# JunkyByte/easy_ViTPose

Measured on AMD Instinct MI355X. Metric: persons_per_sec, higher is better.
Workload: dtype fp16; 1 GPU; ViTPose-B coco K=17, batch 256 x 256x192 crops per GPU (f32 input resident in HBM) -> (y,x,conf) keypoints in HBM; global_batch=256, weights=seeded random init (no checkpoint offline)

## Files before the change

### easy_vitpose_amd/csrc/debug_taps.hip

```cpp
#include "api_internal.h"

using namespace vpi;

namespace {
vp_ctx* dbg_ctx(int device, int dtype) {
    int ndev = 0;
    if (hipGetDeviceCount(&ndev) != hipSuccess || device < 0 || device >= ndev) {
        g_create_error = "no HIP device available (no CPU fallback)";
        return nullptr;
    }
    if (hipSetDevice(device) != hipSuccess) return nullptr;
    vp_ctx* c = new vp_ctx();
    c->cfg.device_id = device;
    c->dtype = dtype == VP_DTYPE_F16 ? vp::DT_F16 : vp::DT_BF16;
    apply_gemm_tuning(c->sw);
    return c;
}
int dbg_finish(vp_ctx* c, int rc) {
    if (rc) g_create_error = c->err;
    vp_destroy(c);
    return rc;
}
int download16(vp_ctx* c, const uint16_t* d, float* out, size_t n) {
    std::vector<uint16_t> t(n);
// ... 274 lines not shown
    if ((r = dalloc(c, &dA, (size_t)M * K)) || (r = dalloc(c, &dW, wrows * K)) || (r = dalloc(c, &c->zero, (size_t)256))) return r;
    vp::fill_random16(c->dtype, dA, (size_t)M * K, 1u, nullptr);
    vp::fill_random16(c->dtype, dW, wrows * K, 2u, nullptr);
    if (flags & 64) { HIPCHK(c, hipMemset(dA, 0, (size_t)M * K * 2)); HIPCHK(c, hipMemset(dW, 0, wrows * K * 2)); }
    if (flags & 128) { HIPCHK(c, hipMemsetD16(dA, 0x3c00, (size_t)M * K)); HIPCHK(c, hipMemsetD16(dW, 0x3c00, wrows * K)); }
    std::vector<float> hb(wrows), hs(wrows), hr((size_t)M * 2);
    uint32_t lcg = 12345u;
    auto rnd = [&]() { lcg = lcg * 1664525u + 1013904223u; return (float)((lcg >> 8) & 0xffff) / 65536.f - 0.5f; };
    for (auto& v : hb) v = rnd();
    for (auto& v : hs) v = 4.f * rnd();
    for (size_t i = 0; i < (size_t)M; ++i) { hr[2 * i] = 0.2f * rnd(); hr[2 * i + 1] = 1.f + 0.4f * rnd(); }
    if ((r = upload_f32(c, &dB, hb.data(), wrows))) return r;
    vp::GemmArgs& g = rc.g;
    g.A = dA; g.W = dW; g.bias = dB; g.M = M; g.N = N; g.K = K; g.ldo = N; g.zero = c->zero; g.Kp = c->Kp;
    g.w_rows = (int)wrows;
    g.persist = (flags & 1) != 0; g.out_blocked = (flags & 2) != 0; g.a_blocked = (flags & 4) != 0; g.reverse = (flags & 8) != 0;
    if (flags & 16) {
        if ((r = upload_f32(c, &dRow, hr.data(), (size_t)M * 2)) || (r = upload_f32(c, &dS, hs.data(), wrows))) return r;
        g.rowstat = dRow; g.ln_s = dS;
    }
    if (epi == vp::EPI_BIAS || epi == vp::EPI_BIAS_GELU) {
        rc.out_bytes = MN * 2;
    } else if (epi == vp::EPI_BIAS_RESID || epi == vp::EPI_POS) {
        rc.out_bytes = MN * 4;
        const size_t na = epi == vp::EPI_BIAS_RESID ? MN : (size_t)192 * N;
        if ((r = dalloc(c, &dAux32, na))) return r;
        std::vector<float> ha(na);
        for (auto& v : ha) v = 2.f * rnd();
        HIPCHK(c, hipMemcpy(dAux32, ha.data(), na * 4, hipMemcpyHostToDevice));
        g.aux = dAux32;
    } else if (epi == vp::EPI_BIAS_RESID_LN) {
// ... 42 lines not shown
        for (size_t m = 0; m < (size_t)M; ++m)
            for (size_t k = 0; k < (size_t)K; ++k) {
                const size_t dst = ablk ? ((((m >> 6) * (K >> 6) + (k >> 6)) << 12) + ((m & 63) << 6) + (k & 63)) : m * K + k;
                ha[dst] = host_to_bits(A[m * K + k], c->dtype);
            }
        if ((r = dalloc(c, &dA, (size_t)M * K))) return dbg_finish(c, r);
        if (hipMemcpy(dA, ha.data(), ha.size() * 2, hipMemcpyHostToDevice) != hipSuccess) return dbg_finish(c, fail(c, VP_ERR_HIP, "H2D"));
    }
    size_t fin_rows = 0;
    if (epi == vp::EPI_HEATMAP) { if ((r = upload_final(c, &dW, W, N, K, &fin_rows))) return dbg_finish(c, r); }
    else if ((r = upload_mat(c, &dW, W, N, K, wrows))) return dbg_finish(c, r);
    if ((r = upload_f32(c, &dB, bias, N, wrows)) || (r = dalloc(c, &c->zero, (size_t)256))) return dbg_finish(c, r);
    vp::GemmArgs g{};
    g.A = dA; g.W = dW; g.bias = dB; g.M = M; g.N = N; g.K = K; g.ldo = N; g.zero = c->zero; g.Kp = N;
    g.w_rows = (int)wrows; g.variant = variant; g.group_m = group_m;
    g.persist = (flags & 1) != 0; g.out_blocked = oblk; g.a_blocked = ablk; g.reverse = (flags & 8) != 0;
    if (rowstat && ln_s) {
        if ((r = upload_f32(c, &dRow, rowstat, (size_t)M * 2)) || (r = upload_f32(c, &dS, ln_s, N, wrows))) return dbg_finish(c, r);
        g.rowstat = dRow; g.ln_s = dS;
    }
    size_t out_bytes = 0;
    const bool prod = epi == vp::EPI_BIAS_RESID_LN || epi == vp::EPI_POS_LN;
    if (epi == vp::EPI_BIAS || epi == vp::EPI_BIAS_GELU) out_bytes = MN * 2;
    else if (epi == vp::EPI_BIAS_RESID || epi == vp::EPI_POS || prod) out_bytes = MN * 4;
    else if (epi == vp::EPI_HEATMAP) { out_bytes = MN * 4; g.N = (int)fin_rows; g.ldo = 0; g.w_rows = (int)pad128(fin_rows); }
    else return dbg_finish(c, fail(c, VP_ERR_INVALID, "unsupported epilogue"));
    if (epi == vp::EPI_BIAS_RESID || epi == vp::EPI_POS || epi == vp::EPI_POS_LN) {
        if (!aux) return dbg_finish(c, fail(c, VP_ERR_INVALID, "aux required"));
        if ((r = upload_f32(c, &dAux32, aux, epi == vp::EPI_BIAS_RESID ? MN : (size_t)192 * N))) return dbg_finish(c, r);
        g.aux = dAux32;
    }
// ... 342 lines not shown
```

### easy_vitpose_amd/csrc/gemm.hip

```cpp
#include <cstdio>
#include <cstdlib>
#include <type_traits>
#include <utility>

#include "common.h"
#include "kernels.h"

namespace vp {

template <int BM_, int BN_, int BK_, int WM_, int WN_, int STAGES_, int PIPE_ = 0, int DIRECT_ = 0>
struct TileCfg {
    static constexpr int DIRECT = DIRECT_;
    static constexpr int BM = BM_, BN = BN_, BK = BK_, WM = WM_, WN = WN_, STAGES = STAGES_;
    static constexpr int PIPE = PIPE_;
    static constexpr int NWM = BM / WM, NWN = BN / WN, NWAVES = NWM * NWN, NT = NWAVES * 64;
    static constexpr int ROWB = BK * 2;
    static constexpr int SLOTS = ROWB / 16;
    static constexpr int RPG = 1024 / ROWB;
    static constexpr int W_BYTES = BN * ROWB, A_BYTES = BM * ROWB, STAGE_BYTES = W_BYTES + A_BYTES;
    static constexpr int LDS = STAGES * STAGE_BYTES;
    static constexpr int WP = BN / RPG / NWAVES, AP = BM / RPG / NWAVES;
    static constexpr int G = WP + AP;
    static constexpr int KK = BK / 32, TI = WN / 16, TJ = WM / 16;
    static_assert(BK == 64 || BK == 32, "BK");
// ... 21 lines not shown
}

__device__ __forceinline__ float row8_sum(float x) {
    x += __builtin_bit_cast(float, __builtin_amdgcn_update_dpp(0, __builtin_bit_cast(int, x), 0xB1, 0xF, 0xF, true));
    x += __builtin_bit_cast(float, __builtin_amdgcn_update_dpp(0, __builtin_bit_cast(int, x), 0x4E, 0xF, 0xF, true));
    x += __builtin_bit_cast(float, __builtin_amdgcn_update_dpp(0, __builtin_bit_cast(int, x), 0x141, 0xF, 0xF, true));
    return x;
}

template <class C> constexpr int epi_rows_per_pass_ln() {
    int jp = C::TJ;
    while (jp > 1 && C::NWM * jp * 16 * (C::BN * 4 + 16) + C::BM * (C::BN / 64) * 8 > C::LDS) jp /= 2;
    return jp;
}

template <int OFF> __device__ __forceinline__ void lds_read_b128(u32x4& d, uint32_t addr) {
    asm volatile("ds_read_b128 %0, %1 offset:%2" : "=v"(d) : "v"(addr), "n"(OFF));
}
template <int N> __device__ __forceinline__ void wait_lgkm() {
    asm volatile("s_waitcnt lgkmcnt(%0)" ::"n"(N));
    __builtin_amdgcn_sched_barrier(0);
}
template <int ROWB, int... Is>
__device__ __forceinline__ void lds_read_frags(u32x4* d, uint32_t addr, std::integer_sequence<int, Is...>) {
    (lds_read_b128<Is * 16 * ROWB>(d[Is], addr), ...);
}

template <int N> __device__ __forceinline__ void wait_vmcnt() {
    asm volatile("s_waitcnt vmcnt(%0)" ::"n"(N) : "memory");
}
// ... 20 lines not shown
    }
}

template <class T, class C, int J>
__device__ __forceinline__ void pipe5_half1(f32x4 (&acc)[C::TI][C::TJ], u32x4* f1) {
    if constexpr (J < C::TJ) {
        wait_lgkm<C::TJ - J - 1>();
#pragma unroll
        for (int i = 0; i < C::TI; ++i) acc[i][J] = mfma16<T>(f1[i], f1[C::TI + J], acc[i][J]);
        __builtin_amdgcn_sched_barrier(0);
        pipe5_half1<T, C, J + 1>(acc, f1);
    }
}

template <class T, int EPI_, int AMODE, class C, bool EXPERT = false>
__global__ __launch_bounds__(C::NT, 2) void gemm_kernel(GemmArgs g) {
    constexpr bool LN_PROD = (EPI_ == EPI_BIAS_RESID_LN || EPI_ == EPI_POS_LN);
    constexpr int EPI = LN_PROD ? EPI_ - 4 : EPI_;
    extern __shared__ __attribute__((aligned(16))) char smem[];
    const int tid = threadIdx.x, lane = tid & 63, wave = tid >> 6;
    const int tiles_n = (g.N + C::BN - 1) / C::BN;
    const int tiles_m = (g.M + C::BM - 1) / C::BM;
    int bid, parity = 0, split = 0;
    if (AMODE == A_DECONV && g.parity_fast) {
        const int lb = xcd_remap(blockIdx.x, tiles_m * tiles_n * 4);
        parity = lb & 3;
        bid = lb >> 2;
    } else if (EPI_ == EPI_PARTIAL) {
        const int lb = xcd_remap(blockIdx.x, tiles_m * tiles_n * g.splitk);
        split = lb / (tiles_m * tiles_n);
        bid = lb - split * (tiles_m * tiles_n);
    } else {
        bid = xcd_remap(blockIdx.x, tiles_m * tiles_n);
        if (AMODE == A_DECONV) parity = blockIdx.y;
    }
    if (g.reverse) bid = tiles_m * tiles_n - 1 - bid;
    int tm, tn;
    if (g.group_m > 1) {
        const int per_group = g.group_m * tiles_n;
        const int grp = bid / per_group, first_m = grp * g.group_m;
        const int gsz = min(tiles_m - first_m, g.group_m);
        const int r = bid - grp * per_group;
        tm = first_m + r % gsz;
        tn = r / gsz;
    } else {
        tm = bid / tiles_n;
        tn = bid - tm * tiles_n;
    }
    const int n0 = tn * C::BN, m0 = tm * C::BM;
    if constexpr (EXPERT) {
        const int e = g.expert[m0 / 192];
        g.W += (size_t)e * g.w_rows * g.K;
        g.bias += (size_t)e * g.w_rows;
    }
    const int K = g.K;
    const int klen = (EPI_ == EPI_PARTIAL) ? K / g.splitk : K;
    const int kbase = (EPI_ == EPI_PARTIAL) ? split * klen : 0;
    if constexpr (LN_PROD) {
        if (VP_STAGGER(g) > 0 && blockIdx.x < 512) {
            const int mode = VP_STAGGER(g) / 1000, n = VP_STAGGER(g) % 1000;
            const uint32_t hw = __builtin_amdgcn_s_getreg((31 << 11) | (0 << 6) | 4);
            bool late;
            if (mode == 0) late = (hw >> 1) & 1;
            else if (mode == 1) late = blockIdx.x >= 256;
            else if (mode == 3) late = (hw >> 8) & 1;
            else if (mode == 4) late = blockIdx.x & 1;
            else if (mode == 5) late = (hw >> 13) & 1;
            else late = (blockIdx.x >> 3) & 1;
            if (late) for (int i = 0; i < n; ++i) __builtin_amdgcn_s_sleep(16);
        }
    }

    const int rip = lane / C::SLOTS, pslot = lane % C::SLOTS;
    const uint16_t* wsrc[C::WP];
    const uint16_t* asrc[C::AP];
    int ai[C::AP], aj[C::AP];
    const uint16_t* W = g.W + (AMODE == A_DECONV ? (size_t)parity * g.w_parity_stride : 0);
#pragma unroll
    for (int p = 0; p < C::WP; ++p) {
        const int r = (p * C::NWAVES + wave) * C::RPG + rip;
        wsrc[p] = W + (size_t)(n0 + r) * K + swz<C::BK>(r, pslot) * 8;
    }
#pragma unroll
    for (int p = 0; p < C::AP; ++p) {
        const int r = (p * C::NWAVES + wave) * C::RPG + rip;
        int m = ((VP_ABLATE(g) & 2) ? 0 : m0) + r;
        if (m > g.M - 1) m = g.M - 1;
        const int sl = swz<C::BK>(r, pslot) * 8;
        if (AMODE == A_DENSE) {
            asrc[p] = g.a_blocked ? g.A + ((size_t)(m >> 6) * (K >> 6) << 12) + ((m & 63) << 6) + sl : g.A + (size_t)m * K + sl;
        } else {
            const int t = m / g.Win;
            ai[p] = t % g.Hin;
            aj[p] = m - t * g.Win;
            asrc[p] = g.A + (size_t)m * g.Cin + sl;
        }
    }
    auto stage = [&](int kt, int buf) {
        char* base = smem + buf * C::STAGE_BYTES + wave * 1024;
        const int k0 = kbase + kt * C::BK;
#pragma unroll
        for (int p = 0; p < C::WP; ++p) glds16(wsrc[p] + k0, base + p * (C::NWAVES * 1024));
        if (AMODE == A_DENSE) {
            const int ka = g.a_blocked ? ((k0 >> 6) << 12) + (k0 & 63) : k0;
#pragma unroll
            for (int p = 0; p < C::AP; ++p) glds16(asrc[p] + ka, base + C::W_BYTES + p * (C::NWAVES * 1024));
        } else {
            const int tap = k0 / g.Cin, c0 = k0 - tap * g.Cin;
            const int ti = tap >> 1, tj = tap & 1;
            const int pa = parity >> 1, pb = parity & 1;
            const int di = pa ? (ti ? 0 : 1) : (ti ? -1 : 0);
            const int dj = pb ? (tj ? 0 : 1) : (tj ? -1 : 0);
#pragma unroll
            for (int p = 0; p < C::AP; ++p) {
                const bool ok = (unsigned)(ai[p] + di) < (unsigned)g.Hin && (unsigned)(aj[p] + dj) < (unsigned)g.Win;
                const uint16_t* src = ok ? asrc[p] + (ptrdiff_t)(di * g.Win + dj) * g.Cin + c0 : g.zero + pslot * 8;
                glds16(src, base + C::W_BYTES + p * (C::NWAVES * 1024));
            }
        }
    };

    const int wn = wave / C::NWM, wm = wave % C::NWM;
    const int frow = lane & 15, fg = lane >> 4;
    const int foff = frow * C::ROWB + (swz<C::BK>(frow, fg) << 4);
    const int woff = wn * C::WN * C::ROWB + foff;
    const int aoff = C::W_BYTES + wm * C::WM * C::ROWB + foff;

    f32x4 acc[C::TI][C::TJ];
#pragma unroll
    for (int i = 0; i < C::TI; ++i)
#pragma unroll
        for (int j = 0; j < C::TJ; ++j) acc[i][j] = f32x4{0.f, 0.f, 0.f, 0.f};

    const int nk = klen / C::BK;
    if constexpr (C::PIPE == 2) {
        static_assert(C::KK == 1 && C::STAGES >= 3, "PIPE 2 needs BK = 32 and >= 3 stages");
        u32x4 wfA[C::TI], afA[C::TJ], wfB[C::TI], afB[C::TJ];
        auto ldfrag = [&](u32x4(&wf)[C::TI], u32x4(&af)[C::TJ], int b) {
            const char* sb = smem + b * C::STAGE_BYTES;
#pragma unroll
            for (int i = 0; i < C::TI; ++i) wf[i] = *(const u32x4*)(sb + (woff + i * 16 * C::ROWB));
#pragma unroll
            for (int j = 0; j < C::TJ; ++j) af[j] = *(const u32x4*)(sb + (aoff + j * 16 * C::ROWB));
        };
        auto settle = [&](u32x4(&wf)[C::TI], u32x4(&af)[C::TJ]) {
#pragma unroll
            for (int i = 0; i < C::TI; ++i) asm volatile("" ::"v"(wf[i]));
#pragma unroll
            for (int j = 0; j < C::TJ; ++j) asm volatile("" ::"v"(af[j]));
// ... 75 lines not shown
                for (int j = 0; j < C::TJ; ++j) acc[i][j] = mfma16<T>(wf[i], af[j], acc[i][j]);
            __builtin_amdgcn_s_setprio(0);
            asm volatile("" ::: "memory");
            __builtin_amdgcn_s_barrier();
            asm volatile("" ::: "memory");
            rbuf = (rbuf + 1) & 3;
            pbuf = (pbuf + 1) & 3;
        }
        if (!grp_b) {
            __builtin_amdgcn_s_barrier();
            asm volatile("" ::: "memory");
        }
    } else {
    constexpr int KS = (C::PIPE == 6) ? 2 : 1;
    static_assert(C::PIPE != 6 || (C::STAGES >= 4 && C::KK == 2), "PIPE 6: >= 4 stages, BK = 64");
#pragma unroll
    for (int s = 0; s < C::STAGES - KS; ++s)
        if (s < nk) stage(s, s);
    if constexpr (EPI == EPI_BIAS || EPI == EPI_BIAS_GELU) {
        if (g.ln_part) {
            float2* st = (float2*)(smem + C::LDS);
            for (int r = tid; r < C::BM; r += C::NT) {
                int m = m0 + r;
                if (m > g.M - 1) m = g.M - 1;
                const float* src = g.ln_part + (size_t)m * g.ln_tiles * 2;
                float mean = 0.f, rstd = 1.f;
                switch (g.ln_tiles) {
                    case 6: ln_merge_row<6>(src, g.ln_inv_d, mean, rstd); break;
                    case 12: ln_merge_row<12>(src, g.ln_inv_d, mean, rstd); break;
                    case 16: ln_merge_row<16>(src, g.ln_inv_d, mean, rstd); break;
                    case 20: ln_merge_row<20>(src, g.ln_inv_d, mean, rstd); break;
                    default: ln_merge(src, g.ln_tiles, g.ln_inv_d, mean, rstd);
                }
                st[r] = float2{mean, rstd};
            }
        }
    }
    int buf = 0, pbuf = C::STAGES - KS;
    for (int kt = 0; kt < nk; kt += KS) {
        if (C::STAGES > 2 * KS && kt + C::STAGES - KS <= nk) wait_vmcnt<C::G * (C::STAGES - 2 * KS)>();
        else wait_vmcnt<0>();
        __builtin_amdgcn_s_barrier();
        asm volatile("" ::: "memory");
#pragma unroll
        for (int ks = 0; ks < KS; ++ks) {
            const int pb = pbuf + ks >= C::STAGES ? pbuf + ks - C::STAGES : pbuf + ks;
            if (kt + C::STAGES - KS + ks < nk && !(VP_ABLATE(g) & 1)) stage(kt + C::STAGES - KS + ks, pb);
        }
#pragma unroll
        for (int ks = 0; ks < KS; ++ks) {
        const int cbuf = buf + ks >= C::STAGES ? buf + ks - C::STAGES : buf + ks;
        const char* sb = smem + cbuf * C::STAGE_BYTES;
        if constexpr (C::PIPE == 5) {
            static_assert(C::KK == 2 && C::TI + C::TJ <= 12 && 2 * C::TJ >= C::TI + C::TJ, "PIPE 5 schedule");
            constexpr int R = C::TI + C::TJ;
            u32x4 f0[R], f1[R];
            const uint32_t lb = (uint32_t)(size_t)(lds_ptr_t)(smem) + cbuf * C::STAGE_BYTES;
            const uint32_t wa0 = lb + woff, wa1 = lb + (woff ^ 64), aa0 = lb + aoff, aa1 = lb + (aoff ^ 64);
            lds_read_frags<C::ROWB>(f0, wa0, std::make_integer_sequence<int, C::TI>{});
            lds_read_frags<C::ROWB>(f0 + C::TI, aa0, std::make_integer_sequence<int, C::TJ>{});
            __builtin_amdgcn_s_setprio(1);
            __builtin_amdgcn_sched_barrier(0);
// ... 123 lines not shown
                float* orow = g.out2 + ((size_t)im * g.Kp + nb) * opix + px;
#pragma unroll
                for (int r = 0; r < 4; ++r)
                    if (im >= 0 && nb + r < g.Kp) orow[(size_t)r * opix] = v[r] + b2[r];
            }
        };
        for (int u = 0; u < groups; u += 2) {
            if (u + 1 < groups) ldw(wB, u + 1);
            group(wA, u);
            if (u + 1 < groups) {
                if (u + 2 < groups) ldw(wA, u + 2);
                group(wB, u + 1);
            }
        }
    } else if constexpr (LN_PROD && !C::DIRECT) {
        constexpr int ROWBYTES = C::BN * 4 + 16;
        constexpr int JP = epi_rows_per_pass_ln<C>();
        constexpr int CR = C::NWM * JP * 16;
        constexpr int CPR = C::BN / 8;
        constexpr int NCH = CR * CPR / C::NT;
        constexpr int GR = C::BN / 64;
        static_assert(NCH * C::NT == CR * CPR && CPR % 8 == 0 && C::NT % 8 == 0, "chunks must split evenly over threads");
        static_assert(CR * ROWBYTES + C::BM * GR * 8 <= C::LDS, "row statistics must fit behind the staged rows");
        float* statbuf = (float*)(smem + CR * ROWBYTES);
        uint16_t* out_hi = (uint16_t*)g.out;
        uint16_t* out_lo = out_hi + g.plane;
        const uint16_t* aux_hi = (const uint16_t*)g.aux;
        const uint16_t* aux_lo = aux_hi + g.plane;
        f32x4 bias4[C::TI];
#pragma unroll
        for (int i = 0; i < C::TI; ++i)
            bias4[i] = (EPI == EPI_POS) ? f32x4{0.f, 0.f, 0.f, 0.f} : *(const f32x4*)(g.bias + n0 + wn * C::WN + i * 16 + fg * 4);
        asm volatile("s_waitcnt vmcnt(0)" ::: "memory");
        __syncthreads();
#pragma unroll
        for (int p = 0; p < C::TJ / JP; ++p) {
            size_t orow_q[NCH];
            u32x4 ra[NCH], rb[NCH];
#pragma unroll
            for (int q = 0; q < NCH; ++q) {
                const int c = tid + q * C::NT;
                const int lr = c / CPR, ch = c - lr * CPR;
                const int wmr = lr / (JP * 16), rr = lr - wmr * (JP * 16);
                const int m = m0 + wmr * C::WM + p * JP * 16 + rr;
                const int n = n0 + ch * 8;
                orow_q[q] = (size_t)-1;
                if (m >= g.M || n >= g.N) continue;
                orow_q[q] = (size_t)m * g.ldo;
                if (EPI == EPI_POS) {
                    const float* pr = g.aux + (size_t)(m % 192) * g.ldo + n;
                    ra[q] = *(const u32x4*)pr;
                    rb[q] = *(const u32x4*)(pr + 4);
                } else {
                    ra[q] = *(const u32x4*)(aux_hi + orow_q[q] + n);
                    rb[q] = *(const u32x4*)(aux_lo + orow_q[q] + n);
                }
            }
#pragma unroll
            for (int jj = 0; jj < JP; ++jj) {
                char* lrow = smem + ((wm * JP + jj) * 16 + frow) * ROWBYTES + (wn * C::WN + fg * 4) * 4;
#pragma unroll
                for (int i = 0; i < C::TI; ++i) *(f32x4*)(lrow + i * 64) = acc[i][p * JP + jj] + bias4[i];
            }
            __syncthreads();
#pragma unroll
            for (int q = 0; q < NCH; ++q) {
                const int c = tid + q * C::NT;
                const int lr = c / CPR, ch = c - lr * CPR;
                const bool ok = orow_q[q] != (size_t)-1;
                float v[8];
#pragma unroll
                for (int e = 0; e < 8; ++e) v[e] = 0.f;
                if (ok) {
                    const f32x4 s0 = *(const f32x4*)(smem + lr * ROWBYTES + ch * 32);
                    const f32x4 s1 = *(const f32x4*)(smem + lr * ROWBYTES + ch * 32 + 16);
#pragma unroll
                    for (int e = 0; e < 8; ++e) {
                        const float st = e < 4 ? s0[e] : s1[e - 4];
                        float r;
                        if (EPI == EPI_POS) {
                            r = __builtin_bit_cast(float, e < 4 ? ra[q][e] : rb[q][e - 4]);
                        } else {
                            const int sh = (e & 1) * 16;
                            r = from_bits<T>((uint16_t)(ra[q][e >> 1] >> sh)) + from_bits<T>((uint16_t)(rb[q][e >> 1] >> sh));
                        }
                        v[e] = st + r;
                    }
                    u32x4 oh, ol;
#pragma unroll
                    for (int e = 0; e < 8; e += 2) { uint32_t h_, l_; split_planes2<T>(v[e], v[e + 1], h_, l_); oh[e >> 1] = h_; ol[e >> 1] = l_; }
                    if (!(VP_ABLATE(g) & 8)) {
                        *(u32x4*)(out_hi + orow_q[q] + n0 + ch * 8) = oh;
                        *(u32x4*)(out_lo + orow_q[q] + n0 + ch * 8) = ol;
                    }
                }
                float s1 = ((v[0] + v[1]) + (v[2] + v[3])) + ((v[4] + v[5]) + (v[6] + v[7]));
                s1 = row8_sum(s1);
                const float mg = s1 * (1.0f / 64.0f);
                float s2 = 0.f;
#pragma unroll
                for (int e = 0; e < 8; ++e) {
                    const float d = v[e] - mg;
                    s2 = fmaf(d, d, s2);
                }
                s2 = row8_sum(s2);
                if ((ch & 7) == 0) {
                    const int wmr = lr / (JP * 16), rr = lr - wmr * (JP * 16);
                    const int trow = wmr * C::WM + p * JP * 16 + rr;
                    *(float2*)(statbuf + (trow * GR + (ch >> 3)) * 2) = float2{s1, s2};
                }
            }
            if (p + 1 < C::TJ / JP) __syncthreads();
        }
        __syncthreads();
        for (int t = tid; t < C::BM * GR; t += C::NT) {
            const int trow = t / GR, gi = t - trow * GR;
            const int m = m0 + trow, n = n0 + gi * 64;
            if (m < g.M && n < g.N && !(VP_ABLATE(g) & 8))
                *(float2*)(g.stats_out + ((size_t)m * (g.N / 64) + (n >> 6)) * 2) = *(const float2*)(statbuf + t * 2);
        }
    } else if constexpr (EPI != EPI_HEATMAP && !C::DIRECT) {
        constexpr int ES = (EPI == EPI_BIAS_RESID || EPI == EPI_POS || EPI == EPI_PARTIAL) ? 4 : 2;
        constexpr int ROWBYTES = C::BN * ES + 16;
        constexpr int JP = epi_rows_per_pass<C, ES>();
        constexpr int CR = C::NWM * JP * 16;
        constexpr int CPR = C::BN * ES / 16;
        constexpr int EPC = 16 / ES;
        constexpr int NCH = CR * CPR / C::NT;
        static_assert(NCH * C::NT == CR * CPR, "chunks must split evenly over threads");
        f32x4 bias4[C::TI];
// ... 159 lines not shown
                    if (EPI == EPI_DECONV) {
#pragma unroll
                        for (int r = 0; r < 4; ++r) v[r] = fmaxf(v[r], 0.f);
                    }
                    u32x2 o;
                    o[0] = pack2<T>(v[0], v[1]);
                    o[1] = pack2<T>(v[2], v[3]);
                    *(u32x2*)((uint16_t*)g.out + orow + nb) = o;
                } else if (EPI == EPI_BIAS_RESID) {
                    *(f32x4*)((float*)g.out + orow + nb) = v + *(const f32x4*)(g.aux + orow + nb);
                } else {
                    *(f32x4*)((float*)g.out + orow + nb) = v + *(const f32x4*)(g.aux + (size_t)(m % 192) * g.ldo + nb);
                }
            }
        }
    }
}

template <class T, int EPI, class C>
__global__ __launch_bounds__(C::NT, 2) void gemm_persist_kernel(GemmArgs g) {
    static_assert(C::BK == 64 && C::STAGES == 2 && C::PIPE == 1 && (EPI == EPI_BIAS || EPI == EPI_BIAS_GELU), "persistent variant");
    extern __shared__ __attribute__((aligned(16))) char smem[];
    const int tid = threadIdx.x, lane = tid & 63, wave = __builtin_amdgcn_readfirstlane(tid >> 6);
    const int tiles_n = (g.N + C::BN - 1) / C::BN;
    const int tiles_m = (g.M + C::BM - 1) / C::BM;
    const int ntiles = tiles_m * tiles_n;
    const int K = g.K, nk = K / C::BK;
    const int xcd = blockIdx.x & 7, j0 = blockIdx.x >> 3, nloc = gridDim.x >> 3;
    const int q = ntiles >> 3, r8 = ntiles & 7;
    const int base = (xcd < r8) ? xcd * (q + 1) : r8 * (q + 1) + (xcd - r8) * q;
// ... 194 lines not shown
            st[0] = ts0; st[1] = ts1; st[2] = __builtin_readcyclecounter();
#pragma unroll
            for (int e = 0; e < 5; ++e) st[3 + e] = ks[e];
        }
        if (!has_next) break;
        t += nloc;
        m0 = nm0;
        n0 = nn0;
        landed = true;
    }
}

template <class T, int EPI, class C>
static hipError_t launch_persist(const GemmArgs& a, hipStream_t s) {
    auto kern = gemm_persist_kernel<T, EPI, C>;
    static bool attr_done[64] = {};
    int dev = 0;
    (void)hipGetDevice(&dev);
    if (dev < 0 || dev >= 64 || !attr_done[dev]) {
        hipError_t e = hipFuncSetAttribute((const void*)kern, hipFuncAttributeMaxDynamicSharedMemorySize, C::LDS);
        if (e != hipSuccess) return e;
        if (dev >= 0 && dev < 64) attr_done[dev] = true;
    }
    const int tiles = ((a.M + C::BM - 1) / C::BM) * ((a.N + C::BN - 1) / C::BN);
    const int resident = 256 * (160 * 1024 / C::LDS);
    int grid = tiles < resident ? tiles : resident;
    grid &= ~7;
    if (grid < 8) return hipErrorInvalidValue;
    if (a.desc)
        snprintf(a.desc, a.desc_cap, "gemm_persist_kernel<%s, %d, TileCfg<%d, %d, %d, %d, %d, %d, %d, %d>>", std::is_same<T, F16>::value ? "F16" : "BF16", EPI,
// ... 49 lines not shown
    if (C::PIPE == 6 && a.K % 128 != 0) return hipErrorInvalidValue;
    if (a.ln_part && (a.ln_tiles & 1)) return hipErrorInvalidValue;
    static bool attr_done[2][64] = {};
    int dev = 0;
    (void)hipGetDevice(&dev);
    if (dev < 0 || dev >= 64 || !attr_done[ex][dev]) {
        hipError_t e = hipFuncSetAttribute((const void*)kern, hipFuncAttributeMaxDynamicSharedMemorySize, LDS_BYTES + LN_STAT_BYTES);
        if (e != hipSuccess) return e;
        if (dev >= 0 && dev < 64) attr_done[ex][dev] = true;
    }
    GemmArgs g = a;
    const int tiles_n = (a.N + C::BN - 1) / C::BN;
    g.w_parity_stride = (size_t)a.w_rows * a.K;
    if ((size_t)tiles_n * C::BN > (size_t)a.w_rows) return hipErrorInvalidValue;
    const int tiles = ((a.M + C::BM - 1) / C::BM) * tiles_n;
    if constexpr (EPI == EPI_PARTIAL) {
        if (a.splitk < 1 || a.K % (a.splitk * C::BK * (C::PIPE == 6 ? 2 : 1)) != 0 || a.ldo != a.N || a.N % 4 != 0 || C::DIRECT || C::PIPE == 2 || C::PIPE == 3) return hipErrorInvalidValue;
    }
    dim3 grid(AMODE == A_DECONV && a.parity_fast ? tiles * 4 : (EPI == EPI_PARTIAL ? tiles * a.splitk : tiles), AMODE == A_DECONV && !a.parity_fast ? 4 : 1);
    if (a.desc)
        snprintf(a.desc, a.desc_cap, "gemm_kernel<%s, %d, %d, TileCfg<%d, %d, %d, %d, %d, %d, %d, %d>%s>", std::is_same<T, F16>::value ? "F16" : "BF16", EPI,
                 AMODE, C::BM, C::BN, C::BK, C::WM, C::WN, C::STAGES, C::PIPE, C::DIRECT, ex ? ", true" : "");
    hipLaunchKernelGGL(kern, grid, dim3(C::NT), LDS_BYTES + (a.ln_part ? LN_STAT_BYTES : 0), s, g);
    return hipGetLastError();
}

#ifdef VP_TOOLS
#define VP_TOOLS_CASE(v) case v: return launch<T, EPI, AMODE, Cfg##v>(a, s);
#else
#define VP_TOOLS_CASE(v)
#endif
template <class T, int EPI, int AMODE>
static hipError_t by_variant(const GemmArgs& a, hipStream_t s) {
    switch (a.variant) {
// ... 85 lines not shown
            GemmArgs b = a;
            b.stagger = stagger_env;
            return gemm8_launch(dtype, epi, b, a.variant == 17 ? 192 : 256, s, a.variant == 18 ? 192 : 256);
        }
#endif
        return gemm8_launch(dtype, epi, a, a.variant == 17 ? 192 : 256, s, a.variant == 18 ? 192 : 256);
    }
#ifdef VP_TOOLS
    static const int proj_stagger_env = [] { const char* e = getenv("VP_PROJ_STAGGER"); return e ? atoi(e) : 0; }();
    if (proj_stagger_env > 0 && (epi == EPI_BIAS_RESID_LN) && a.K <= a.N) {
        GemmArgs b = a;
        b.stagger = proj_stagger_env;
        return dtype == DT_F16 ? dispatch<F16>(epi, b, s) : dispatch<BF16>(epi, b, s);
    }
#endif
    if (a.persist) {
        if ((epi != EPI_BIAS && epi != EPI_BIAS_GELU) || a.variant != 8 || a.K % 128 || a.N % 8 || a.ldo != a.N || a.reverse ||
            a.M % Cfg8::BM || (size_t)a.M * a.K * 2 >= (1ull << 32) ||
            (size_t)((a.N + Cfg8::BN - 1) / Cfg8::BN) * Cfg8::BN > (size_t)a.w_rows)
            return hipErrorInvalidValue;
        if (dtype == DT_F16)
            return epi == EPI_BIAS ? launch_persist<F16, EPI_BIAS, Cfg8>(a, s) : launch_persist<F16, EPI_BIAS_GELU, Cfg8>(a, s);
        return epi == EPI_BIAS ? launch_persist<BF16, EPI_BIAS, Cfg8>(a, s) : launch_persist<BF16, EPI_BIAS_GELU, Cfg8>(a, s);
    }
    if (a.a_blocked && (epi == EPI_DECONV || epi == EPI_DECONV_FINAL || (a.M & 63))) return hipErrorInvalidValue;
    if (a.out_blocked && ((epi != EPI_BIAS && epi != EPI_BIAS_GELU) || (a.M & 63) || (a.N & 63) || a.ldo != a.N)) return hipErrorInvalidValue;
    if ((epi == EPI_BIAS_RESID_LN || epi == EPI_POS_LN) && (a.N % 64 != 0 || !a.plane || !a.stats_out)) return hipErrorInvalidValue;
    return dtype == DT_F16 ? dispatch<F16>(epi, a, s) : dispatch<BF16>(epi, a, s);
}

// ... 2 lines not shown
```

### easy_vitpose_amd/csrc/kernels.h

```cpp
#pragma once
#include <hip/hip_runtime.h>
#include <stdint.h>

#ifdef VP_TOOLS
#define VP_ABLATE(g) ((g).ablate)
#define VP_STAGGER(g) ((g).stagger)
#else
#define VP_ABLATE(g) 0
#define VP_STAGGER(g) 0
#endif

namespace vp {

enum { DT_F16 = 0, DT_BF16 = 1 };

enum GemmEpi {
    EPI_BIAS = 0,
    EPI_BIAS_GELU = 1,
    EPI_BIAS_RESID = 2,
    EPI_POS = 3,
    EPI_DECONV = 4,
    EPI_HEATMAP = 5,
    EPI_BIAS_RESID_LN = 6,
    EPI_POS_LN = 7,
// ... 18 lines not shown
    float* out2;
    int w_rows;
    int variant;
    int group_m;
    size_t w_parity_stride;
    size_t plane;
    float* stats_out;
    const float* rowstat;
    const float* ln_s;
    const float* ln_part;
    int ln_tiles;
    float ln_inv_d;
    int a_blocked, out_blocked;
    int reverse;
    int persist;
    int stagger;
    int ablate;
    char* desc;
    int desc_cap;
    float attn_scale_log2e;
    int splitk;
    int parity_fast;
    union {
        const uint8_t* a_scales;
        const int32_t* expert;
    };
    const float* w_scale;
    uint8_t* out_scales;
};
hipError_t gemm_launch(int dtype, int epi, const GemmArgs& a, hipStream_t s);
// ... 76 lines not shown
```

Measured before the change: 25460 persons/s.

## Loop residual-LN GEMM blocks over multiple tiles, prefetching next tile during epilogue

For the bias+residual+LayerNorm-producing GEMM configuration, launches a resident-sized grid where each block walks several output tiles and issues the first K-stage load of the next tile before running the current tile's epilogue. The epilogue is moved into the second LDS stage so it does not collide with the prefetched stage, and the residual loads are double-buffered across chunks. It also raises the launch-bounds occupancy hint for 8-wave configs. The aim is to hide per-tile prologue latency and epilogue memory stalls, at the cost of more register pressure and more complex control flow.

```diff
diff --git a/easy_vitpose_amd/csrc/debug_taps.hip b/easy_vitpose_amd/csrc/debug_taps.hip
--- a/easy_vitpose_amd/csrc/debug_taps.hip
+++ b/easy_vitpose_amd/csrc/debug_taps.hip
@@ -312,7 +312,7 @@
     vp::GemmArgs& g = rc.g;
     g.A = dA; g.W = dW; g.bias = dB; g.M = M; g.N = N; g.K = K; g.ldo = N; g.zero = c->zero; g.Kp = c->Kp;
     g.w_rows = (int)wrows;
-    g.persist = (flags & 1) != 0; g.out_blocked = (flags & 2) != 0; g.a_blocked = (flags & 4) != 0; g.reverse = (flags & 8) != 0;
+    g.persist = (flags & 1) != 0; g.out_blocked = (flags & 2) != 0; g.a_blocked = (flags & 4) != 0; g.reverse = (flags & 8) != 0; g.one_tile = (flags & 32) != 0;
     if (flags & 16) {
         if ((r = upload_f32(c, &dRow, hr.data(), (size_t)M * 2)) || (r = upload_f32(c, &dS, hs.data(), wrows))) return r;
         g.rowstat = dRow; g.ln_s = dS;
@@ -385,7 +385,7 @@
     vp::GemmArgs g{};
     g.A = dA; g.W = dW; g.bias = dB; g.M = M; g.N = N; g.K = K; g.ldo = N; g.zero = c->zero; g.Kp = N;
     g.w_rows = (int)wrows; g.variant = variant; g.group_m = group_m;
-    g.persist = (flags & 1) != 0; g.out_blocked = oblk; g.a_blocked = ablk; g.reverse = (flags & 8) != 0;
+    g.persist = (flags & 1) != 0; g.out_blocked = oblk; g.a_blocked = ablk; g.reverse = (flags & 8) != 0; g.one_tile = (flags & 32) != 0;
     if (rowstat && ln_s) {
         if ((r = upload_f32(c, &dRow, rowstat, (size_t)M * 2)) || (r = upload_f32(c, &dS, ln_s, N, wrows))) return dbg_finish(c, r);
         g.rowstat = dRow; g.ln_s = dS;
diff --git a/easy_vitpose_amd/csrc/gemm.hip b/easy_vitpose_amd/csrc/gemm.hip
--- a/easy_vitpose_amd/csrc/gemm.hip
+++ b/easy_vitpose_amd/csrc/gemm.hip
@@ -59,6 +59,11 @@
     return jp;
 }
 
+template <class C, int EPI_, int AMODE, bool EXPERT> constexpr bool ln_tile_loop_cfg() {
+    return EPI_ == EPI_BIAS_RESID_LN && AMODE == A_DENSE && !EXPERT && !C::DIRECT && C::BK == 64 && C::STAGES == 2 && C::PIPE <= 1 &&
+           C::NWM * epi_rows_per_pass_ln<C>() * 16 * (C::BN * 4 + 16) + C::BM * (C::BN / 64) * 8 <= C::STAGE_BYTES;
+}
+
 template <int OFF> __device__ __forceinline__ void lds_read_b128(u32x4& d, uint32_t addr) {
     asm volatile("ds_read_b128 %0, %1 offset:%2" : "=v"(d) : "v"(addr), "n"(OFF));
 }
@@ -109,11 +114,11 @@
 }
 
 template <class T, int EPI_, int AMODE, class C, bool EXPERT = false>
-__global__ __launch_bounds__(C::NT, 2) void gemm_kernel(GemmArgs g) {
+__global__ __launch_bounds__(C::NT, (ln_tile_loop_cfg<C, EPI_, AMODE, EXPERT>() && C::NWAVES == 8) ? 4 : 2) void gemm_kernel(GemmArgs g) {
     constexpr bool LN_PROD = (EPI_ == EPI_BIAS_RESID_LN || EPI_ == EPI_POS_LN);
     constexpr int EPI = LN_PROD ? EPI_ - 4 : EPI_;
     extern __shared__ __attribute__((aligned(16))) char smem[];
-    const int tid = threadIdx.x, lane = tid & 63, wave = tid >> 6;
+    const int tid = threadIdx.x, lane = tid & 63, wave = ln_tile_loop_cfg<C, EPI_, AMODE, EXPERT>() ? __builtin_amdgcn_readfirstlane(tid >> 6) : tid >> 6;
     const int tiles_n = (g.N + C::BN - 1) / C::BN;
     const int tiles_m = (g.M + C::BM - 1) / C::BM;
     int bid, parity = 0, split = 0;
@@ -129,20 +134,35 @@
         bid = xcd_remap(blockIdx.x, tiles_m * tiles_n);
         if (AMODE == A_DECONV) parity = blockIdx.y;
     }
-    if (g.reverse) bid = tiles_m * tiles_n - 1 - bid;
-    int tm, tn;
-    if (g.group_m > 1) {
-        const int per_group = g.group_m * tiles_n;
-        const int grp = bid / per_group, first_m = grp * g.group_m;
-        const int gsz = min(tiles_m - first_m, g.group_m);
-        const int r = bid - grp * per_group;
-        tm = first_m + r % gsz;
-        tn = r / gsz;
-    } else {
-        tm = bid / tiles_n;
-        tn = bid - tm * tiles_n;
-    }
-    const int n0 = tn * C::BN, m0 = tm * C::BM;
+    constexpr bool LOOPABLE = ln_tile_loop_cfg<C, EPI_, AMODE, EXPERT>();
+    int lt = 0, lstep = 0, lcnt = 0, lbase = 0;
+    if constexpr (LOOPABLE) {
+        if (g.tile_loop) {
+            lt = blockIdx.x >> 3;
+            lstep = gridDim.x >> 3;
+            lbase = xcd_remap(blockIdx.x & 7, tiles_m * tiles_n);
+            lcnt = ((tiles_m * tiles_n) >> 3) + ((int)(blockIdx.x & 7) < ((tiles_m * tiles_n) & 7) ? 1 : 0);
+        }
+    }
+    auto tile_origin = [&](int b, int& m0_, int& n0_) {
+        if (g.reverse) b = tiles_m * tiles_n - 1 - b;
+        int tm, tn;
+        if (g.group_m > 1) {
+            const int per_group = g.group_m * tiles_n;
+            const int grp = b / per_group, first_m = grp * g.group_m;
+            const int gsz = min(tiles_m - first_m, g.group_m);
+            const int r = b - grp * per_group;
+            tm = first_m + r % gsz;
+            tn = r / gsz;
+        } else {
+            tm = b / tiles_n;
+            tn = b - tm * tiles_n;
+        }
+        m0_ = tm * C::BM;
+        n0_ = tn * C::BN;
+    };
+    int n0, m0;
+    tile_origin(bid, m0, n0);
     if constexpr (EXPERT) {
         const int e = g.expert[m0 / 192];
         g.W += (size_t)e * g.w_rows * g.K;
@@ -171,26 +191,36 @@
     const uint16_t* asrc[C::AP];
     int ai[C::AP], aj[C::AP];
     const uint16_t* W = g.W + (AMODE == A_DECONV ? (size_t)parity * g.w_parity_stride : 0);
-#pragma unroll
-    for (int p = 0; p < C::WP; ++p) {
-        const int r = (p * C::NWAVES + wave) * C::RPG + rip;
-        wsrc[p] = W + (size_t)(n0 + r) * K + swz<C::BK>(r, pslot) * 8;
-    }
-#pragma unroll
-    for (int p = 0; p < C::AP; ++p) {
-        const int r = (p * C::NWAVES + wave) * C::RPG + rip;
-        int m = ((VP_ABLATE(g) & 2) ? 0 : m0) + r;
-        if (m > g.M - 1) m = g.M - 1;
-        const int sl = swz<C::BK>(r, pslot) * 8;
-        if (AMODE == A_DENSE) {
-            asrc[p] = g.a_blocked ? g.A + ((size_t)(m >> 6) * (K >> 6) << 12) + ((m & 63) << 6) + sl : g.A + (size_t)m * K + sl;
-        } else {
-            const int t = m / g.Win;
-            ai[p] = t % g.Hin;
-            aj[p] = m - t * g.Win;
-            asrc[p] = g.A + (size_t)m * g.Cin + sl;
-        }
-    }
+    auto set_addr = [&](int m0_, int n0_) {
+        int rip = lane / C::SLOTS, pslot = lane % C::SLOTS;
+        if constexpr (LOOPABLE) {
+            int l = __builtin_amdgcn_mbcnt_hi(~0u, __builtin_amdgcn_mbcnt_lo(~0u, 0u));
+            asm volatile("" : "+v"(l));
+            rip = l / C::SLOTS;
+            pslot = l % C::SLOTS;
+        }
+#pragma unroll
+        for (int p = 0; p < C::WP; ++p) {
+            const int r = (p * C::NWAVES + wave) * C::RPG + rip;
+            wsrc[p] = W + (size_t)(n0_ + r) * K + swz<C::BK>(r, pslot) * 8;
+        }
+#pragma unroll
+        for (int p = 0; p < C::AP; ++p) {
+            const int r = (p * C::NWAVES + wave) * C::RPG + rip;
+            int m = ((VP_ABLATE(g) & 2) ? 0 : m0_) + r;
+            if (m > g.M - 1) m = g.M - 1;
+            const int sl = swz<C::BK>(r, pslot) * 8;
+            if (AMODE == A_DENSE) {
+                asrc[p] = g.a_blocked ? g.A + ((size_t)(m >> 6) * (K >> 6) << 12) + ((m & 63) << 6) + sl : g.A + (size_t)m * K + sl;
+            } else {
+                const int t = m / g.Win;
+                ai[p] = t % g.Hin;
+                aj[p] = m - t * g.Win;
+                asrc[p] = g.A + (size_t)m * g.Cin + sl;
+            }
+        }
+    };
+    set_addr(m0, n0);
     auto stage = [&](int kt, int buf) {
         char* base = smem + buf * C::STAGE_BYTES + wave * 1024;
         const int k0 = kbase + kt * C::BK;
@@ -221,13 +251,20 @@
     const int woff = wn * C::WN * C::ROWB + foff;
     const int aoff = C::W_BYTES + wm * C::WM * C::ROWB + foff;
 
+    const int nk = klen / C::BK;
+    bool landed = false;
+    for (;;) {
+    bool has_next = false;
+    int nm0 = 0, nn0 = 0;
+    if constexpr (LOOPABLE) {
+        if (landed) set_addr(m0, n0);
+    }
     f32x4 acc[C::TI][C::TJ];
 #pragma unroll
     for (int i = 0; i < C::TI; ++i)
 #pragma unroll
         for (int j = 0; j < C::TJ; ++j) acc[i][j] = f32x4{0.f, 0.f, 0.f, 0.f};
 
-    const int nk = klen / C::BK;
     if constexpr (C::PIPE == 2) {
         static_assert(C::KK == 1 && C::STAGES >= 3, "PIPE 2 needs BK = 32 and >= 3 stages");
         u32x4 wfA[C::TI], afA[C::TJ], wfB[C::TI], afB[C::TJ];
@@ -333,9 +370,11 @@
     } else {
     constexpr int KS = (C::PIPE == 6) ? 2 : 1;
     static_assert(C::PIPE != 6 || (C::STAGES >= 4 && C::KK == 2), "PIPE 6: >= 4 stages, BK = 64");
-#pragma unroll
-    for (int s = 0; s < C::STAGES - KS; ++s)
-        if (s < nk) stage(s, s);
+    if (!landed) {
+#pragma unroll
+        for (int s = 0; s < C::STAGES - KS; ++s)
+            if (s < nk) stage(s, s);
+    }
     if constexpr (EPI == EPI_BIAS || EPI == EPI_BIAS_GELU) {
         if (g.ln_part) {
             float2* st = (float2*)(smem + C::LDS);
@@ -358,13 +397,26 @@
     int buf = 0, pbuf = C::STAGES - KS;
     for (int kt = 0; kt < nk; kt += KS) {
         if (C::STAGES > 2 * KS && kt + C::STAGES - KS <= nk) wait_vmcnt<C::G * (C::STAGES - 2 * KS)>();
-        else wait_vmcnt<0>();
+        else if (!(LOOPABLE && landed && kt == 0)) wait_vmcnt<0>();
         __builtin_amdgcn_s_barrier();
         asm volatile("" ::: "memory");
 #pragma unroll
         for (int ks = 0; ks < KS; ++ks) {
             const int pb = pbuf + ks >= C::STAGES ? pbuf + ks - C::STAGES : pbuf + ks;
             if (kt + C::STAGES - KS + ks < nk && !(VP_ABLATE(g) & 1)) stage(kt + C::STAGES - KS + ks, pb);
+        }
+        if constexpr (LOOPABLE) {
+            if (kt + 1 == nk && lt + lstep < lcnt) {
+                has_next = true;
+                tile_origin(lbase + lt + lstep, nm0, nn0);
+                const ptrdiff_t dw = (ptrdiff_t)(nn0 - n0) * K;
+                const ptrdiff_t da = (VP_ABLATE(g) & 2) ? 0 : g.a_blocked ? (ptrdiff_t)((nm0 - m0) / 64) * (K >> 6) * 4096 : (ptrdiff_t)(nm0 - m0) * K;
+#pragma unroll
+                for (int p = 0; p < C::WP; ++p) wsrc[p] += dw;
+#pragma unroll
+                for (int p = 0; p < C::AP; ++p) asrc[p] += da;
+                stage(0, 0);
+            }
         }
 #pragma unroll
         for (int ks = 0; ks < KS; ++ks) {
@@ -518,6 +570,13 @@
             }
         }
     } else if constexpr (LN_PROD && !C::DIRECT) {
+        int lane_e = lane;
+        if constexpr (LOOPABLE) {
+            lane_e = __builtin_amdgcn_mbcnt_hi(~0u, __builtin_amdgcn_mbcnt_lo(~0u, 0u));
+            asm volatile("" : "+v"(lane_e));
+        }
+        const int wave_e = wave, tid_e = wave_e * 64 + lane_e;
+        const int wn_e = wave_e / C::NWM, wm_e = wave_e % C::NWM, frow_e = lane_e & 15, fg_e = lane_e >> 4;
         constexpr int ROWBYTES = C::BN * 4 + 16;
         constexpr int JP = epi_rows_per_pass_ln<C>();
         constexpr int CR = C::NWM * JP * 16;
@@ -526,7 +585,8 @@
         constexpr int GR = C::BN / 64;
         static_assert(NCH * C::NT == CR * CPR && CPR % 8 == 0 && C::NT % 8 == 0, "chunks must split evenly over threads");
         static_assert(CR * ROWBYTES + C::BM * GR * 8 <= C::LDS, "row statistics must fit behind the staged rows");
-        float* statbuf = (float*)(smem + CR * ROWBYTES);
+        char* const cst = smem + (LOOPABLE ? C::STAGE_BYTES : 0);
+        float* statbuf = (float*)(cst + CR * ROWBYTES);
         uint16_t* out_hi = (uint16_t*)g.out;
         uint16_t* out_lo = out_hi + g.plane;
         const uint16_t* aux_hi = (const uint16_t*)g.aux;
@@ -534,68 +594,89 @@
         f32x4 bias4[C::TI];
 #pragma unroll
         for (int i = 0; i < C::TI; ++i)
-            bias4[i] = (EPI == EPI_POS) ? f32x4{0.f, 0.f, 0.f, 0.f} : *(const f32x4*)(g.bias + n0 + wn * C::WN + i * 16 + fg * 4);
-        asm volatile("s_waitcnt vmcnt(0)" ::: "memory");
-        __syncthreads();
-#pragma unroll
-        for (int p = 0; p < C::TJ / JP; ++p) {
-            size_t orow_q[NCH];
-            u32x4 ra[NCH], rb[NCH];
-#pragma unroll
-            for (int q = 0; q < NCH; ++q) {
-                const int c = tid + q * C::NT;
+            bias4[i] = (EPI == EPI_POS) ? f32x4{0.f, 0.f, 0.f, 0.f} : *(const f32x4*)(g.bias + n0 + wn_e * C::WN + i * 16 + fg_e * 4);
+        if constexpr (LOOPABLE) {
+            asm volatile("s_waitcnt lgkmcnt(0)" ::: "memory");
+            __builtin_amdgcn_s_barrier();
+            asm volatile("" ::: "memory");
+        } else {
+            asm volatile("s_waitcnt vmcnt(0)" ::: "memory");
+            __syncthreads();
+        }
+        constexpr int NP = C::TJ / JP;
+        auto load_chunk = [&](int p, int q, size_t& orow, u32x4& ra, u32x4& rb) {
+            {
+                const int c = tid_e + q * C::NT;
                 const int lr = c / CPR, ch = c - lr * CPR;
                 const int wmr = lr / (JP * 16), rr = lr - wmr * (JP * 16);
                 const int m = m0 + wmr * C::WM + p * JP * 16 + rr;
                 const int n = n0 + ch * 8;
-                orow_q[q] = (size_t)-1;
-                if (m >= g.M || n >= g.N) continue;
-                orow_q[q] = (size_t)m * g.ldo;
+                if constexpr (LOOPABLE) {
+                    const size_t o = (size_t)min(m, g.M - 1) * g.ldo + min(n, g.N - 8);
+                    ra = *(const u32x4*)(aux_hi + o);
+                    rb = *(const u32x4*)(aux_lo + o);
+                    return;
+                }
+                orow = (size_t)-1;
+                if (m >= g.M || n >= g.N) return;
+                orow = (size_t)m * g.ldo;
                 if (EPI == EPI_POS) {
                     const float* pr = g.aux + (size_t)(m % 192) * g.ldo + n;
-                    ra[q] = *(const u32x4*)pr;
-                    rb[q] = *(const u32x4*)(pr + 4);
+                    ra = *(const u32x4*)pr;
+                    rb = *(const u32x4*)(pr + 4);
                 } else {
-                    ra[q] = *(const u32x4*)(aux_hi + orow_q[q] + n);
-                    rb[q] = *(const u32x4*)(aux_lo + orow_q[q] + n);
-                }
-            }
+                    ra = *(const u32x4*)(aux_hi + orow + n);
+                    rb = *(const u32x4*)(aux_lo + orow + n);
+                }
+            }
+        };
+        auto stage_pass = [&](int p) {
 #pragma unroll
             for (int jj = 0; jj < JP; ++jj) {
-                char* lrow = smem + ((wm * JP + jj) * 16 + frow) * ROWBYTES + (wn * C::WN + fg * 4) * 4;
-#pragma unroll
-                for (int i = 0; i < C::TI; ++i) *(f32x4*)(lrow + i * 64) = acc[i][p * JP + jj] + bias4[i];
-            }
-            __syncthreads();
-#pragma unroll
-            for (int q = 0; q < NCH; ++q) {
-                const int c = tid + q * C::NT;
+                char* lrow = cst + ((wm_e * JP + jj) * 16 + frow_e) * ROWBYTES + (wn_e * C::WN + fg_e * 4) * 4;
+#pragma unroll
+                for (int i = 0; i < C::TI; ++i) *(f32x4*)(lrow + i * 64) = LOOPABLE ? acc[i][p * JP + jj] : acc[i][p * JP + jj] + bias4[i];
+            }
+        };
+        auto finish_chunk = [&](int p, int q, const size_t orow_q, const u32x4& ra, const u32x4& rb) {
+            {
+                const int c = tid_e + q * C::NT;
                 const int lr = c / CPR, ch = c - lr * CPR;
-                const bool ok = orow_q[q] != (size_t)-1;
+                bool ok;
+                size_t orow;
+                if constexpr (LOOPABLE) {
+                    const int wmr = lr / (JP * 16), rr = lr - wmr * (JP * 16);
+                    const int m = m0 + wmr * C::WM + p * JP * 16 + rr;
+                    ok = m < g.M && n0 + ch * 8 < g.N;
+                    orow = (size_t)m * g.ldo;
+                } else {
+                    ok = orow_q != (size_t)-1;
+                    orow = orow_q;
+                }
                 float v[8];
 #pragma unroll
                 for (int e = 0; e < 8; ++e) v[e] = 0.f;
-                if (ok) {
-                    const f32x4 s0 = *(const f32x4*)(smem + lr * ROWBYTES + ch * 32);
-                    const f32x4 s1 = *(const f32x4*)(smem + lr * ROWBYTES + ch * 32 + 16);
+                if (LOOPABLE || ok) {
+                    const f32x4 s0 = *(const f32x4*)(cst + lr * ROWBYTES + ch * 32);
+                    const f32x4 s1 = *(const f32x4*)(cst + lr * ROWBYTES + ch * 32 + 16);
 #pragma unroll
                     for (int e = 0; e < 8; ++e) {
                         const float st = e < 4 ? s0[e] : s1[e - 4];
                         float r;
                         if (EPI == EPI_POS) {
-                            r = __builtin_bit_cast(float, e < 4 ? ra[q][e] : rb[q][e - 4]);
+                            r = __builtin_bit_cast(float, e < 4 ? ra[e] : rb[e - 4]);
                         } else {
                             const int sh = (e & 1) * 16;
-                            r = from_bits<T>((uint16_t)(ra[q][e >> 1] >> sh)) + from_bits<T>((uint16_t)(rb[q][e >> 1] >> sh));
+                            r = from_bits<T>((uint16_t)(ra[e >> 1] >> sh)) + from_bits<T>((uint16_t)(rb[e >> 1] >> sh));
                         }
                         v[e] = st + r;
                     }
                     u32x4 oh, ol;
 #pragma unroll
                     for (int e = 0; e < 8; e += 2) { uint32_t h_, l_; split_planes2<T>(v[e], v[e + 1], h_, l_); oh[e >> 1] = h_; ol[e >> 1] = l_; }
-                    if (!(VP_ABLATE(g) & 8)) {
-                        *(u32x4*)(out_hi + orow_q[q] + n0 + ch * 8) = oh;
-                        *(u32x4*)(out_lo + orow_q[q] + n0 + ch * 8) = ol;
+                    if (ok && !(VP_ABLATE(g) & 8)) {
+                        *(u32x4*)(out_hi + orow + n0 + ch * 8) = oh;
+                        *(u32x4*)(out_lo + orow + n0 + ch * 8) = ol;
                     }
                 }
                 float s1 = ((v[0] + v[1]) + (v[2] + v[3])) + ((v[4] + v[5]) + (v[6] + v[7]));
@@ -614,10 +695,44 @@
                     *(float2*)(statbuf + (trow * GR + (ch >> 3)) * 2) = float2{s1, s2};
                 }
             }
-            if (p + 1 < C::TJ / JP) __syncthreads();
+        };
+        if constexpr (LOOPABLE) {
+            size_t unused = 0;
+            u32x4 ra[2], rb[2];
+            load_chunk(0, 0, unused, ra[0], rb[0]);
+#pragma unroll
+            for (int i = 0; i < C::TI; ++i)
+#pragma unroll
+                for (int j = 0; j < C::TJ; ++j) acc[i][j] = acc[i][j] + bias4[i];
+#pragma unroll
+            for (int p = 0; p < NP; ++p) {
+                stage_pass(p);
+                if (p == 0) wait_vmcnt<0>();
+                __syncthreads();
+#pragma unroll
+                for (int q = 0; q < NCH; ++q) {
+                    const int cur = p * NCH + q, nxt = cur + 1;
+                    if (nxt < NP * NCH) load_chunk(nxt / NCH, nxt % NCH, unused, ra[nxt & 1], rb[nxt & 1]);
+                    finish_chunk(p, q, unused, ra[cur & 1], rb[cur & 1]);
+                }
+                if (p + 1 < NP) __syncthreads();
+            }
+        } else {
+#pragma unroll
+            for (int p = 0; p < NP; ++p) {
+                size_t orow_q[NCH];
+                u32x4 ra[NCH], rb[NCH];
+#pragma unroll
+                for (int q = 0; q < NCH; ++q) load_chunk(p, q, orow_q[q], ra[q], rb[q]);
+                stage_pass(p);
+                __syncthreads();
+#pragma unroll
+                for (int q = 0; q < NCH; ++q) finish_chunk(p, q, orow_q[q], ra[q], rb[q]);
+                if (p + 1 < NP) __syncthreads();
+            }
         }
         __syncthreads();
-        for (int t = tid; t < C::BM * GR; t += C::NT) {
+        for (int t = tid_e; t < C::BM * GR; t += C::NT) {
             const int trow = t / GR, gi = t - trow * GR;
             const int m = m0 + trow, n = n0 + gi * 64;
             if (m < g.M && n < g.N && !(VP_ABLATE(g) & 8))
@@ -807,6 +922,16 @@
                 }
             }
         }
+    }
+    if constexpr (LOOPABLE) {
+        if (!has_next) break;
+        lt += lstep;
+        m0 = nm0;
+        n0 = nn0;
+        landed = true;
+    } else {
+        break;
+    }
     }
 }
 
@@ -1031,6 +1156,7 @@
 template <class T, int EPI, class C>
 static hipError_t launch_persist(const GemmArgs& a, hipStream_t s) {
     auto kern = gemm_persist_kernel<T, EPI, C>;
+    if (a.ln_part) return hipErrorInvalidValue;
     static bool attr_done[64] = {};
     int dev = 0;
     (void)hipGetDevice(&dev);
@@ -1110,10 +1236,19 @@
     g.w_parity_stride = (size_t)a.w_rows * a.K;
     if ((size_t)tiles_n * C::BN > (size_t)a.w_rows) return hipErrorInvalidValue;
     const int tiles = ((a.M + C::BM - 1) / C::BM) * tiles_n;
+    int grid_x = tiles;
+    g.tile_loop = 0;
+    if constexpr (ln_tile_loop_cfg<C, EPI, AMODE, false>()) {
+        constexpr int resident = 256 * (160 * 1024 / C::LDS);
+        if (!a.one_tile && !a.expert && tiles > resident && a.M % C::BM == 0 && a.N % C::BN == 0 && a.K % (2 * C::BK) == 0) {
+            g.tile_loop = 1;
+            grid_x = resident;
+        }
+    }
     if constexpr (EPI == EPI_PARTIAL) {
         if (a.splitk < 1 || a.K % (a.splitk * C::BK * (C::PIPE == 6 ? 2 : 1)) != 0 || a.ldo != a.N || a.N % 4 != 0 || C::DIRECT || C::PIPE == 2 || C::PIPE == 3) return hipErrorInvalidValue;
     }
-    dim3 grid(AMODE == A_DECONV && a.parity_fast ? tiles * 4 : (EPI == EPI_PARTIAL ? tiles * a.splitk : tiles), AMODE == A_DECONV && !a.parity_fast ? 4 : 1);
+    dim3 grid(AMODE == A_DECONV && a.parity_fast ? tiles * 4 : (EPI == EPI_PARTIAL ? tiles * a.splitk : grid_x), AMODE == A_DECONV && !a.parity_fast ? 4 : 1);
     if (a.desc)
         snprintf(a.desc, a.desc_cap, "gemm_kernel<%s, %d, %d, TileCfg<%d, %d, %d, %d, %d, %d, %d, %d>%s>", std::is_same<T, F16>::value ? "F16" : "BF16", EPI,
                  AMODE, C::BM, C::BN, C::BK, C::WM, C::WN, C::STAGES, C::PIPE, C::DIRECT, ex ? ", true" : "");
@@ -1229,6 +1364,14 @@
         return dtype == DT_F16 ? dispatch<F16>(epi, b, s) : dispatch<BF16>(epi, b, s);
     }
 #endif
+#ifdef VP_TOOLS
+    static const int ln_loop_env = [] { const char* e = getenv("VP_LN_LOOP"); return e ? atoi(e) : 1; }();
+    if (!ln_loop_env && !a.one_tile && (epi == EPI_BIAS_RESID_LN || epi == EPI_POS_LN)) {
+        GemmArgs b = a;
+        b.one_tile = 1;
+        return gemm_launch(dtype, epi, b, s);
+    }
+#endif
     if (a.persist) {
         if ((epi != EPI_BIAS && epi != EPI_BIAS_GELU) || a.variant != 8 || a.K % 128 || a.N % 8 || a.ldo != a.N || a.reverse ||
             a.M % Cfg8::BM || (size_t)a.M * a.K * 2 >= (1ull << 32) ||
diff --git a/easy_vitpose_amd/csrc/kernels.h b/easy_vitpose_amd/csrc/kernels.h
--- a/easy_vitpose_amd/csrc/kernels.h
+++ b/easy_vitpose_amd/csrc/kernels.h
@@ -56,6 +56,7 @@
     int a_blocked, out_blocked;
     int reverse;
     int persist;
+    int tile_loop, one_tile;
     int stagger;
     int ablate;
     char* desc;
```

Result: no change. 25520 persons/s, median of 6 (+0.2%).
